# Takatsuka-Mark/Photogrammetry

Hardware: AMD Instinct MI355X
Metric: descriptor pairs matched/sec (higher is better)
Workload: dtype u8 / bits (descriptor bits expanded to fp4 +-1 for the MFMA distance: exact integers in f32 accumulators; integer keys); f32 grey; 1 GPU; BASELINE configs[2] (SURVEY 8d config 3) x 1: 64-frame 1920x1080 RGBA64 sequence(s), dewarp(shipped coeffs)+gray+FAST(T=0.1)+NMS(r=16; SURVEY 8d writes r = 20 for this config: both leave more than 4096 survivors per frame, the lists are cut to the same length either way)+BRIEF-256 per frame, all 2016 ordered image pairs per sequence through the greedy Hamming match, <=4096 keypoints per frame (fir; frames=64, image_pairs=2016, frames_per_gpu=64, image_pairs_per_gpu=2016, parallelism=frames f mod 1, image pairs p mod 1; 2 all-gathers per step (elided at N = 1), jobs_in_flight=2, rehearsal_on_one_gpu_with_gloo=False

## Files before the change

### photogrammetry_amd/csrc/k_fast.hip

```cpp
#include "pgx_internal.h"

namespace {

constexpr int TW = 64, TH = 32, HALO = 3;
constexpr int LROWS = TH + 2 * HALO;
constexpr int LSTRIDE = 72;

__global__ __launch_bounds__(256) void k_fast_planes(const float *__restrict__ gray, int W, int H, float T,
                                                     unsigned long long *__restrict__ seg, int ntx,
                                                     uint32_t *__restrict__ segcnt)
{
    __shared__ float tile[LROWS][LSTRIDE];
    __shared__ uint16_t queue[TW * TH];
    __shared__ unsigned planes[TH][3][2];
    __shared__ unsigned qcount;
    const int tx = blockIdx.x, ty = blockIdx.y, f = blockIdx.z;
    const int lane = threadIdx.x & 63, wv = threadIdx.x >> 6;
    const float *g = gray + (size_t)f * W * H;
    const int x0 = tx * TW - HALO, y0 = ty * TH - HALO;
    if (threadIdx.x < TH * 6) (&planes[0][0][0])[threadIdx.x] = 0u;
    if (threadIdx.x == 0) qcount = 0u;

    {
        constexpr int NR = (LROWS + 3) / 4;
        float v[NR], hv[NR];
#pragma unroll
        for (int k = 0; k < NR; k++) {
            const int r = wv + 4 * k;
            const int gy = y0 + r;
            const bool rowok = r < LROWS && gy >= 0 && gy < H;
            const float *grow = g + (size_t)(rowok ? gy : 0) * W;
            const int gx = x0 + lane, hx = x0 + 64 + lane;
            v[k] = (rowok && gx >= 0 && gx < W) ? grow[gx] : 0.0f;
            hv[k] = (rowok && lane < 2 * HALO && hx < W) ? grow[hx] : 0.0f;
        }
#pragma unroll
        for (int k = 0; k < NR; k++) {
            const int r = wv + 4 * k;
            if (r < LROWS) {
                tile[r][lane] = v[k];
                if (lane < 2 * HALO) tile[r][64 + lane] = hv[k];
            }
        }
    }
    __syncthreads();

    const int x = tx * TW + lane;
    const bool xin = x >= 3 && x < W - 3;
#pragma unroll 1
    for (int k = 0; k < TH / 4; k++) {
        const int ry = wv * (TH / 4) + k;
        const int y = ty * TH + ry;
        if (y >= H) break;
        bool pass = false;
        unsigned cb = 0;
        if (xin && y >= 3 && y < H - 3) {
            const float c = tile[ry + 3][lane + 3];
            const float lo = __fsub_rn(c, T), hi = __fadd_rn(c, T);
#define PGX_SIM(dx, dy) ((tile[ry + 3 + (dy)][lane + 3 + (dx)] > lo) & (tile[ry + 3 + (dy)][lane + 3 + (dx)] < hi))
            const unsigned s0 = PGX_SIM(-3, 0), s4 = PGX_SIM(0, 3), s8 = PGX_SIM(3, 0), s12 = PGX_SIM(0, -3);
#undef PGX_SIM
            pass = s0 + s4 + s8 + s12 <= 1u;
            cb = s0 | (s4 << 1) | (s8 << 2) | (s12 << 3);
        }
        const unsigned long long pm = __ballot(pass);
        if (pm) {
            unsigned base = 0;
            if (lane == 0) base = atomicAdd(&qcount, (unsigned)__popcll(pm));
            base = (unsigned)__shfl((int)base, 0);
            if (pass) queue[base + (unsigned)__popcll(pm & ((1ull << lane) - 1ull))] = (uint16_t)((ry << 10) | (lane << 4) | cb);
        }
    }
    __syncthreads();

    const unsigned nq = qcount;
    for (unsigned e = threadIdx.x; e < nq; e += 256) {
        const unsigned q = queue[e];
        const int ry = (int)(q >> 10), lx = (int)((q >> 4) & 63u);
        const float c = tile[ry + 3][lx + 3];
        const float lo = __fsub_rn(c, T), hi = __fadd_rn(c, T);
#define PGX_SIM(dx, dy) ((unsigned)((tile[ry + 3 + (dy)][lx + 3 + (dx)] > lo) & (tile[ry + 3 + (dy)][lx + 3 + (dx)] < hi)))
        unsigned S = (q & 1u) | ((q & 2u) << 3) | ((q & 4u) << 6) | ((q & 8u) << 9);
        const unsigned s1 = PGX_SIM(-3, 1);
        S |= s1 << 1;
        S |= PGX_SIM(-2, 2) << 2;
        S |= PGX_SIM(-1, 3) << 3;
        S |= PGX_SIM(1, 3) << 5;
        S |= PGX_SIM(2, 2) << 6;
        S |= PGX_SIM(3, 1) << 7;
        S |= PGX_SIM(3, -1) << 9;
        S |= PGX_SIM(2, -2) << 10;
        S |= PGX_SIM(1, -3) << 11;
        S |= PGX_SIM(-1, -3) << 13;
        S |= PGX_SIM(-2, -2) << 14;
        S |= s1 << 15;
#undef PGX_SIM
        int score = 0;
        if (S == 0u) {
            score = 16;
        } else {
            const unsigned D = ~S & 0xFFFFu;
            const unsigned dd = D | (D << 16);
            const unsigned x1 = dd & (dd >> 1);
            const unsigned x2 = x1 & (x1 >> 2);
            const unsigned x3 = x2 & (x2 >> 4);
            const unsigned t12 = x3 & (x2 >> 8);
            if (t12) {
                const unsigned t13 = t12 & (dd >> 12);
                const unsigned t14 = t13 & (dd >> 13);
                const unsigned t15 = t14 & (dd >> 14);
                score = 12 + (t13 != 0u) + (t14 != 0u) + (t15 != 0u);
            }
        }
        if (score) {
            const int code = score - 11;
            const unsigned bit = 1u << (lx & 31);
            unsigned *pw = &planes[ry][0][lx >> 5];
            if (code & 1) atomicOr(pw, bit);
            if (code & 2) atomicOr(pw + 2, bit);
            if (code & 4) atomicOr(pw + 4, bit);
        }
    }
    __syncthreads();

    if (threadIdx.x < TH) {
        const int ry = threadIdx.x, y = ty * TH + ry;
        if (y < H) {
            const unsigned long long b0 = planes[ry][0][0] | ((unsigned long long)planes[ry][0][1] << 32);
            const unsigned long long b1 = planes[ry][1][0] | ((unsigned long long)planes[ry][1][1] << 32);
            const unsigned long long b2 = planes[ry][2][0] | ((unsigned long long)planes[ry][2][1] << 32);
            unsigned long long *o = seg + (((size_t)f * H + y) * ntx + tx) * 4;
            *reinterpret_cast<ulonglong2 *>(o) = make_ulonglong2(b0, b1);
            const uint32_t cnt = (uint32_t)__popcll(b0 | b1 | b2);
            *reinterpret_cast<ulonglong2 *>(o + 2) = make_ulonglong2(b2, (unsigned long long)cnt);
            segcnt[((size_t)f * H + y) * ntx + tx] = cnt;
        }
    }
}

__global__ __launch_bounds__(1024) void k_seg_scan(int nseg, uint32_t *__restrict__ segoff, int32_t *__restrict__ n_raw,
                                                   int raw_cap, int *status)
{
    __shared__ uint32_t wsum[16];
    __shared__ uint32_t carry_s;
    const int f = blockIdx.x;
    uint32_t *so = segoff + (size_t)f * nseg;
    const int tid = threadIdx.x, lane = tid & 63, wv = tid >> 6;
    if (tid == 0) carry_s = 0;
    __syncthreads();
    for (int base = 0; base < nseg; base += 1024 * 4) {
        const int i0 = base + tid * 4;
        uint32_t c[4];
        if (i0 + 3 < nseg && (nseg & 3) == 0) {
            const uint4 v = *reinterpret_cast<const uint4 *>(so + i0);
            c[0] = v.x; c[1] = v.y; c[2] = v.z; c[3] = v.w;
        } else {
#pragma unroll
            for (int k = 0; k < 4; k++) c[k] = (i0 + k < nseg) ? so[i0 + k] : 0u;
        }
        uint32_t tsum = c[0] + c[1] + c[2] + c[3];
        uint32_t incl = tsum;
#pragma unroll
        for (int d = 1; d < 64; d <<= 1) {
            uint32_t v = __shfl_up(incl, d);
            if (lane >= d) incl += v;
        }
        if (lane == 63) wsum[wv] = incl;
        __syncthreads();
        uint32_t woff = 0;
        for (int w = 0; w < wv; w++) woff += wsum[w];
        uint32_t run = carry_s + woff + incl - tsum;
#pragma unroll
// ... 14 lines not shown
__global__ __launch_bounds__(256) void k_fast_compact(const unsigned long long *__restrict__ seg,
                                                      const uint32_t *__restrict__ segoff, int H, int ntx,
                                                      uint32_t *__restrict__ raw_xy, int32_t *__restrict__ raw_score,
                                                      int raw_cap)
{
    const int f = blockIdx.y;
    const int nseg = H * ntx;
    const int s = blockIdx.x * 256 + threadIdx.x;
    if (s >= nseg) return;
    const unsigned long long *sg = seg + ((size_t)f * nseg + s) * 4;
    const ulonglong2 p01 = *reinterpret_cast<const ulonglong2 *>(sg);
    const unsigned long long b0 = p01.x, b1 = p01.y, b2 = sg[2];
    unsigned long long any = b0 | b1 | b2;
    if (!any) return;
    uint32_t pos = segoff[(size_t)f * nseg + s];
    const int y = s / ntx, tx = s - y * ntx;
    while (any) {
        const int l = __builtin_ctzll(any);
        any &= any - 1;
        if (pos >= (uint32_t)raw_cap) break;
        const int code = (int)((b0 >> l) & 1ull) | ((int)((b1 >> l) & 1ull) << 1) | ((int)((b2 >> l) & 1ull) << 2);
        raw_xy[(size_t)f * raw_cap + pos] = ((uint32_t)y << 16) | (uint32_t)(tx * 64 + l);
        raw_score[(size_t)f * raw_cap + pos] = code + 11;
        pos++;
    }
}

}

size_t pgx_fast_seg_count(int W, int H) { return (size_t)H * ((W + TW - 1) / TW); }

void pgx_launch_fast(hipStream_t s, const float *gray, int F, int W, int H, float T,
                     unsigned long long *seg, uint32_t *segoff, int32_t *n_raw, uint32_t *raw_xy,
                     int32_t *raw_score, int raw_cap, int *status, bool compact)
{
    if (F <= 0 || W <= 0 || H <= 0) return;
    const int ntx = (W + TW - 1) / TW, nty = (H + TH - 1) / TH;
    const int nseg = H * ntx;
    hipLaunchKernelGGL(k_fast_planes, dim3(ntx, nty, F), dim3(256), 0, s, gray, W, H, T, seg, ntx, segoff);
    hipLaunchKernelGGL(k_seg_scan, dim3(F), dim3(1024), 0, s, nseg, segoff, n_raw, raw_cap, status);
    if (compact)
        hipLaunchKernelGGL(k_fast_compact, dim3((nseg + 255) / 256, F), dim3(256), 0, s, seg, segoff, H, ntx, raw_xy,
                           raw_score, raw_cap);
}
```

### photogrammetry_amd/csrc/k_image.hip

```cpp
#include "pgx_internal.h"

namespace {

__device__ __forceinline__ float gray_of(uint2 px)
{
    float r = (float)(px.x & 0xFFFFu), g = (float)(px.x >> 16), b = (float)(px.y & 0xFFFFu);
    float s = __fadd_rn(__fadd_rn(r, b), g);
    return __fdiv_rn(s, 196605.0f);
}

constexpr int FB = 4;

__device__ __forceinline__ uint2 widen8(uint32_t v)
{
    return make_uint2(__builtin_amdgcn_perm(v, v, 0x01010000u), __builtin_amdgcn_perm(v, v, 0x03030202u));
}

template <bool SRC8> struct SrcPix { using type = uint2; };
template <> struct SrcPix<true> { using type = uint32_t; };
template <bool SRC8> __device__ __forceinline__ uint2 load_px(const typename SrcPix<SRC8>::type *p);
template <> __device__ __forceinline__ uint2 load_px<false>(const uint2 *p) { return *p; }
template <> __device__ __forceinline__ uint2 load_px<true>(const uint32_t *p) { return widen8(*p); }

template <bool HAS_MAP, bool WRITE_RGBA, bool SRC8>
__global__ __launch_bounds__(256) void k_dewarp_gray(const typename SrcPix<SRC8>::type *__restrict__ rgba,
                                                     const int2 *__restrict__ map, int W, int H, int F,
                                                     float *__restrict__ gray, uint2 *__restrict__ dewarped, int *status)
{
    using Px = typename SrcPix<SRC8>::type;
    const size_t npix = (size_t)W * H;
    const int f0 = blockIdx.y * FB;
    const int nf = F - f0 < FB ? F - f0 : FB;
    const size_t ngroups = (npix + 3) / 4;
    const bool vec = (npix & 3) == 0 || F == 1;
    bool oob = false;
    for (size_t grp = (size_t)blockIdx.x * blockDim.x + threadIdx.x; grp < ngroups;
         grp += (size_t)gridDim.x * blockDim.x) {
        const size_t i0 = grp * 4;
        if (vec && i0 + 3 < npix) {
            size_t so[4];
            bool ok[4];
            if (HAS_MAP) {
                const int4 m01 = *reinterpret_cast<const int4 *>(map + i0);
                const int4 m23 = *reinterpret_cast<const int4 *>(map + i0 + 2);
                const int us[4] = {m01.x, m01.z, m23.x, m23.z};
                const int vs[4] = {m01.y, m01.w, m23.y, m23.w};
#pragma unroll
                for (int k = 0; k < 4; k++) {
                    const unsigned su = (unsigned)us[k] & 0xFFFFu, sv = (unsigned)vs[k] & 0xFFFFu;
                    ok[k] = su < (unsigned)W && sv < (unsigned)H;
                    oob |= !ok[k];
                    so[k] = ok[k] ? (size_t)sv * W + su : 0;
                }
            }
            uint2 px[FB][4];
// ... 21 lines not shown
#pragma unroll
                    for (int k = 0; k < 4; k++) if (!ok[k]) px[fb][k] = make_uint2(0, 0);
                }
                if (gray) {
                    const float4 g4 = make_float4(gray_of(px[fb][0]), gray_of(px[fb][1]), gray_of(px[fb][2]), gray_of(px[fb][3]));
                    *reinterpret_cast<float4 *>(gray + (size_t)(f0 + fb) * npix + i0) = g4;
                }
                if (WRITE_RGBA) {
                    uint2 *dout = dewarped + (size_t)(f0 + fb) * npix;
                    *reinterpret_cast<uint4 *>(dout + i0) = make_uint4(px[fb][0].x, px[fb][0].y, px[fb][1].x, px[fb][1].y);
                    *reinterpret_cast<uint4 *>(dout + i0 + 2) = make_uint4(px[fb][2].x, px[fb][2].y, px[fb][3].x, px[fb][3].y);
                }
            }
        } else {
            for (size_t i = i0; i < npix && i < i0 + 4; i++) {
                size_t o = i;
                bool okk = true;
                if (HAS_MAP) {
                    const int2 m = map[i];
                    const unsigned su = (unsigned)m.x & 0xFFFFu, sv = (unsigned)m.y & 0xFFFFu;
                    okk = su < (unsigned)W && sv < (unsigned)H;
                    oob |= !okk;
                    o = okk ? (size_t)sv * W + su : 0;
                }
                for (int fb = 0; fb < nf; fb++) {
                    const uint2 p = okk ? load_px<SRC8>(rgba + (size_t)(f0 + fb) * npix + o) : make_uint2(0, 0);
                    if (gray) gray[(size_t)(f0 + fb) * npix + i] = gray_of(p);
                    if (WRITE_RGBA) dewarped[(size_t)(f0 + fb) * npix + i] = p;
                }
            }
        }
    }
    if (HAS_MAP && oob) atomicOr(status, (int)PGX_ST_OOB_SOURCE);
}

__device__ __forceinline__ int32_t trunc_to_int_dev(double v)
{
    if (!(v > -2147483649.0 && v < 2147483648.0)) return INT32_MIN;
    return (int32_t)v;
}

__device__ __forceinline__ double cbrt_signed_dev(double n)
{
    const double sgn = (double)((n > 0) - (n < 0));
    return pow(fabs(n), 1.0 / 3.0) * sgn;
}

__global__ __launch_bounds__(256) void k_dewarp_map(int W, int H, double k0, double k1, double k2, double k3, double k4,
                                                    int2 *__restrict__ map, int *status)
{
    const size_t i = (size_t)blockIdx.x * 256 + threadIdx.x;
    if (i >= (size_t)W * H) return;
    const int v = (int)(i / W), u = (int)(i - (size_t)v * W);
    const double x0 = W / 2.0, y0 = H / 2.0;
    const int x = trunc_to_int_dev(u - x0), y = trunc_to_int_dev(v - y0);
    const int rd2 = x * x + y * y;
    const double rd = sqrt((double)rd2);
    const double den = rd * k4 - k1;
    const double a2 = (rd * k3 - k0) / den, a1 = (rd * k2 - 1) / den, a0 = rd / den;
    const double Q = (3 * a1 - a2 * a2) / 9.0;
    const double R = (9.0 * a2 * a1 - 27 * a0 - 2 * a2 * a2 * a2) / 54.0;
    const double Q3 = Q * Q * Q;
    const double D = Q3 + R * R;
    const double shift = -a2 / 3.0;
    const double nan = __longlong_as_double(0x7FF8000000000000ll);
    double r0 = nan, r1 = nan, r2 = nan;
// ... 22 lines not shown
        if (kept[0] > kept[1]) { const double t = kept[0]; kept[0] = kept[1]; kept[1] = t; }
    }
    const double root = n == 3 ? kept[1] : kept[0];
    const double theta = atan2((double)y, (double)x);
    map[i] = make_int2(trunc_to_int_dev(root * cos(theta) + x0), trunc_to_int_dev(root * sin(theta) + y0));
}

}

void pgx_launch_dewarp_gray(hipStream_t s, const void *rgba, int src8, const int32_t *map_uv, int F, int W, int H,
                            float *gray, uint16_t *dewarped, int *status)
{
    if (F <= 0 || W <= 0 || H <= 0) return;
    const size_t ngroups = ((size_t)W * H + 3) / 4;
    unsigned gx = (unsigned)((ngroups + 255) / 256);
    const unsigned ny = (unsigned)((F + FB - 1) / FB);
    const unsigned cap = 512u / ny > 32u ? 512u / ny : 32u;
    if (gx > cap) gx = cap;
    dim3 grid(gx, (unsigned)((F + FB - 1) / FB)), block(256);
    const int2 *map = reinterpret_cast<const int2 *>(map_uv);
    uint2 *dw = reinterpret_cast<uint2 *>(dewarped);
#define PGX_DG(M, WR, S8) hipLaunchKernelGGL((k_dewarp_gray<M, WR, S8>), grid, block, 0, s, \
                                             reinterpret_cast<const SrcPix<S8>::type *>(rgba), map, W, H, F, gray, dw, status)
    if (src8) {
        if (map) { if (dw) PGX_DG(true, true, true); else PGX_DG(true, false, true); }
        else { if (dw) PGX_DG(false, true, true); else PGX_DG(false, false, true); }
    } else {
        if (map) { if (dw) PGX_DG(true, true, false); else PGX_DG(true, false, false); }
        else { if (dw) PGX_DG(false, true, false); else PGX_DG(false, false, false); }
    }
#undef PGX_DG
}

void pgx_launch_dewarp_map(hipStream_t s, int W, int H, const double *k, int32_t *map_uv, int *status)
{
    const size_t npix = (size_t)W * H;
    hipLaunchKernelGGL(k_dewarp_map, dim3((unsigned)((npix + 255) / 256)), dim3(256), 0, s, W, H, k[0], k[1], k[2], k[3], k[4],
                       reinterpret_cast<int2 *>(map_uv), status);
}
```

### photogrammetry_amd/csrc/pgx_api.hip

```cpp
#include "pgx_trackgraph.h"
#include "pgx_brief_plan.h"

#include <atomic>
#include <cmath>
#include <cstdarg>
#include <cstdio>
#include <new>
#include <cstring>
#include <cstdlib>

#define PGX_VERSION_STR "pgx 0.1 (gfx950)"

static thread_local std::string tl_err;
static thread_local const pgx_ctx *tl_err_ctx = nullptr;
static thread_local unsigned long long tl_err_id = 0;
static std::atomic<unsigned long long> g_ctx_ids{0};

void pgx_note_error(pgx_ctx *c, const std::string &msg)
{
    tl_err = msg;
    tl_err_ctx = c;
    tl_err_id = c ? c->id : 0;
    if (c) {
        std::lock_guard<std::mutex> g(c->err_mu);
// ... 139 lines not shown
    HIPCHK(c, c->ws_rawxy.ensure((size_t)F * raw_cap * 4));
    HIPCHK(c, c->ws_rawscore.ensure((size_t)F * raw_cap * 4));
    HIPCHK(c, c->ws_nms.ensure((size_t)F * nms_stride));
    const int kp_eff = c->kp_cap <= cap ? c->kp_cap : cap;
    HIPCHK(c, c->ws_order.ensure((size_t)F * kp_eff * 4));
    HIPCHK(c, c->ws_nkept.ensure((size_t)F * 4));
    if (pl.n_levels > 1) {
        HIPCHK(c, c->ws_pyr_cnt.ensure((size_t)16 * F * 4));
        if (pl.n_run > 1) {
            const size_t slots = (size_t)(pl.n_run - 1) * F * kp_eff;
            HIPCHK(c, c->ws_pyr_a.ensure((size_t)F * pl.dims[1][0] * pl.dims[1][1] * 4));
            if (pl.n_run > 2) HIPCHK(c, c->ws_pyr_b.ensure((size_t)F * pl.dims[2][0] * pl.dims[2][1] * 4));
            HIPCHK(c, c->ws_pyr_kp.ensure(slots * sizeof(pgx_keypoint)));
            HIPCHK(c, c->ws_pyr_desc.ensure(slots * c->words * 4));
            if (c->steer_on) HIPCHK(c, c->ws_pyr_bins.ensure(slots * 4));
        }
    }
    return PGX_OK;
}

namespace {

PgxSteer steer_of(const pgx_ctx *c, int32_t *d_bins = nullptr)
{
    return PgxSteer{c->d_steer_pairs.as<int32_t>(), c->d_steer_plans.as<int32_t>(), c->d_steer_dirs.as<int32_t>(), c->steer_B,
                    c->steer_R, d_bins};
}

void enqueue_from_gray(pgx_ctx *c, const float *gray, int F, int W, int H, int kp_eff, bool kp_soft, pgx_keypoint *d_kp,
                       uint32_t *d_desc, int32_t *d_counts, int32_t *d_nraw, int out_stride, int32_t *d_bins)
{
    const int raw_cap = c->raw_cap;
    const size_t nms_stride = pgx_nms_ws_bytes(W, H, c->radius, raw_cap, true);
    {
        ProfScope ps(c, "fast");
        pgx_launch_fast(c->stream, gray, F, W, H, c->threshold, c->ws_seg.as<unsigned long long>(),
                        c->ws_segoff.as<uint32_t>(), d_nraw, c->ws_rawxy.as<uint32_t>(),
                        c->ws_rawscore.as<int32_t>(), raw_cap, c->d_status,
                        !pgx_nms_fills_raw_lists(W, H, c->radius, raw_cap));
    }
    {
        ProfScope ps(c, "nms");
        pgx_launch_nms(c->stream, c->ws_rawxy.as<uint32_t>(), c->ws_rawscore.as<int32_t>(), d_nraw, F, raw_cap, W, H,
                       c->radius, c->ws_nms.p, nms_stride, c->ws_order.as<uint32_t>(), c->ws_nkept.as<int32_t>(),
                       kp_eff, c->d_status, c->ws_seg.as<unsigned long long>(), c->ws_segoff.as<uint32_t>(), kp_soft);
    }
    {
        ProfScope ps(c, "brief");
        const PgxSteer st = steer_of(c, d_bins);
        pgx_launch_brief(c->stream, gray, F, W, H, c->ws_rawxy.as<uint32_t>(), c->ws_rawscore.as<int32_t>(), raw_cap,
                         c->ws_order.as<uint32_t>(), c->ws_nkept.as<int32_t>(), kp_eff, c->d_pairs.as<int32_t>(), c->d_plan.as<int32_t>(), c->P,
                         d_kp, d_desc, d_counts, out_stride, c->steer_on ? &st : nullptr);
    }
}

int enqueue_detect_bins(pgx_ctx *c, const uint16_t *d_rgba, int F, int W, int H, pgx_keypoint *d_kp, uint32_t *d_desc,
                        int32_t *d_counts, int32_t *d_nraw, int cap, int32_t *d_bins, int32_t *d_origin = nullptr,
                        int32_t *d_stats = nullptr)
{
    const int rcp = pgx_prepare_detect(c, F, W, H, cap);
    if (rcp != PGX_OK) return rcp;
    if (F <= 0) return PGX_OK;
    const bool kp_soft = c->kp_cap <= cap;
    const int kp_eff = kp_soft ? c->kp_cap : cap;

    float *gray = c->ws_gray.as<float>();
    {
        ProfScope ps(c, "dewarp_gray");
        pgx_launch_dewarp_gray(c->stream, d_rgba, c->src8, c->map_set ? c->d_map.as<int32_t>() : nullptr, F, W, H, gray,
                               nullptr, c->d_status);
    }
    if (c->pyr_levels <= 1) {
        enqueue_from_gray(c, gray, F, W, H, kp_eff, kp_soft, d_kp, d_desc, d_counts, d_nraw, cap, d_bins);
    } else {
        const PyrPlan pl = pyr_plan(c, W, H);
        int32_t *lvl_counts = c->ws_pyr_cnt.as<int32_t>(), *lvl_nraw = lvl_counts + (size_t)8 * F;
        const size_t lvl_slots = (size_t)F * kp_eff;
        int32_t *tmp_bins = d_bins ? c->ws_pyr_bins.as<int32_t>() : nullptr;
        enqueue_from_gray(c, gray, F, W, H, kp_eff, kp_soft, d_kp, d_desc, lvl_counts, lvl_nraw, cap, d_bins);
        const float *src = gray;
        for (int l = 1; l < pl.n_run; l++) {
            float *dst = (l & 1) ? c->ws_pyr_a.as<float>() : c->ws_pyr_b.as<float>();
            {
                ProfScope ps(c, "pyramid");
                pgx_launch_pyr_down(c->stream, src, F, pl.dims[l - 1][0], pl.dims[l - 1][1], dst, pl.dims[l][0], pl.dims[l][1],
                                    c->pyr_step);
            }
            enqueue_from_gray(c, dst, F, pl.dims[l][0], pl.dims[l][1], kp_eff, kp_soft,
                              c->ws_pyr_kp.as<pgx_keypoint>() + (l - 1) * lvl_slots,
                              c->ws_pyr_desc.as<uint32_t>() + (l - 1) * lvl_slots * c->words, lvl_counts + (size_t)l * F,
                              lvl_nraw + (size_t)l * F, kp_eff, tmp_bins ? tmp_bins + (l - 1) * lvl_slots : nullptr);
            src = dst;
        }
        {
            ProfScope ps(c, "pyramid_append");
            pgx_launch_pyr_append(c->stream, c->ws_pyr_kp.as<pgx_keypoint>(), c->ws_pyr_desc.as<uint32_t>(), tmp_bins, lvl_counts,
                                  lvl_nraw, F, kp_eff, c->words, pl.n_levels, pl.n_run, W, H, pl.scale, d_kp, d_desc, d_bins,
                                  d_counts, d_nraw, d_origin, d_stats, cap, c->d_status);
        }
    }
    HIPCHK(c, hipEventRecord(c->ev_stage[PGX_STAGE_DETECT], c->stream));
    HIPCHK(c, hipGetLastError());
    return PGX_OK;
}
// ... 112 lines not shown
    if (strncmp(prop.gcnArchName, "gfx950", 6) != 0) {
        fprintf(stderr, "pgx: device %d is %s; this library is built for gfx950 only\n", device, prop.gcnArchName);
        return PGX_E_HIP;
    }
    pgx_ctx *c = new (std::nothrow) pgx_ctx();
    if (!c) return PGX_E_HIP;
    c->device = device;
    c->id = ++g_ctx_ids;
    if (hipStreamCreateWithFlags(&c->own_stream, hipStreamNonBlocking) != hipSuccess ||
        hipEventCreateWithFlags(&c->ev_stage[0], hipEventDisableTiming) != hipSuccess ||
        hipEventCreateWithFlags(&c->ev_stage[1], hipEventDisableTiming) != hipSuccess ||
        hipEventCreateWithFlags(&c->ev_stage[2], hipEventDisableTiming) != hipSuccess ||
        hipEventCreateWithFlags(&c->ev_stage[3], hipEventDisableTiming) != hipSuccess ||
        hipMalloc(reinterpret_cast<void **>(&c->d_status), 256) != hipSuccess ||
        hipHostMalloc(reinterpret_cast<void **>(&c->h_status), 64, hipHostMallocDefault) != hipSuccess ||
        hipMemset(c->d_status, 0, 256) != hipSuccess) {
        pgx_ctx_destroy(c);
        return PGX_E_HIP;
    }
    c->stream = c->own_stream;
    *out = c;
    return PGX_OK;
}

void pgx_ctx_destroy(pgx_ctx *c)
{
    if (!c) return;
    (void)hipSetDevice(c->device);
    if (c->stream) (void)hipStreamSynchronize(c->stream);
    if (c->comm) (void)pgx_comm_destroy(c);
    for (auto &kv : c->prof)
        for (auto &ev : kv.second.pending) { (void)hipEventDestroy(ev.first); (void)hipEventDestroy(ev.second); }
    for (hipEvent_t ev : c->ev_pool) (void)hipEventDestroy(ev);
    DevBuf *bufs[] = {&c->d_pairs, &c->d_plan, &c->d_steer_pairs, &c->d_steer_plans, &c->d_steer_dirs, &c->d_map, &c->ws_gray, &c->ws_seg, &c->ws_segoff, &c->ws_nraw, &c->ws_rawxy,
                      &c->ws_rawscore, &c->ws_nms, &c->ws_order, &c->ws_nkept, &c->st_a, &c->st_b, &c->st_c,
                      &c->st_d, &c->st_e, &c->st_f, &c->ws_pose, &c->ws_tracks, &c->ws_tracks_split, &c->ws_agree, &c->ws_matchn[0], &c->ws_matchn[1], &c->ws_matchn[2], &c->ws_knn, &c->ws_guided, &c->ws_tri, &c->ws_ba, &c->ws_reg, &c->ws_ver, &c->ws_init, &c->ws_cns, &c->ws_vocab,
                      &c->ws_pyr_a, &c->ws_pyr_b, &c->ws_pyr_kp, &c->ws_pyr_desc, &c->ws_pyr_bins, &c->ws_pyr_cnt};
    for (DevBuf *b : bufs) b->release();
    c->pin_in.release();
    c->pin_out.release();
    if (c->d_status) (void)hipFree(c->d_status);
    if (c->h_status) (void)hipHostFree(c->h_status);
    for (int k = 0; k < 3; k++) {
        if (c->mstream[k]) (void)hipStreamDestroy(c->mstream[k]);
        if (c->ev_wide[k]) (void)hipEventDestroy(c->ev_wide[k]);
        if (c->ev_rows[k]) (void)hipEventDestroy(c->ev_rows[k]);
        if (c->ev_fin[k]) (void)hipEventDestroy(c->ev_fin[k]);
        if (c->ev_join[k]) (void)hipEventDestroy(c->ev_join[k]);
    }
    if (c->ev_in) (void)hipEventDestroy(c->ev_in);
    for (int k = 0; k < 4; k++) if (c->ev_stage[k]) (void)hipEventDestroy(c->ev_stage[k]);
    if (c->own_stream) (void)hipStreamDestroy(c->own_stream);
    delete c;
}

const char *pgx_last_error(pgx_ctx *c)
{
    if (!c) return "null context";
    if (tl_err_ctx == c && tl_err_id == c->id) return tl_err.c_str();
    static thread_local std::string copy;
    {
        std::lock_guard<std::mutex> g(c->err_mu);
        copy = c->err;
    }
    return copy.c_str();
}

int pgx_set_stream(pgx_ctx *c, void *hip_stream)
{
    if (!c) return PGX_E_BADARG;
    Lock l(c);
    c->cfg_epoch++;
    HIPCHK(c, hipStreamSynchronize(c->stream));
    c->stream = hip_stream ? reinterpret_cast<hipStream_t>(hip_stream) : c->own_stream;
    return PGX_OK;
}

int pgx_check_status(pgx_ctx *c)
{
    if (!c) return PGX_E_BADARG;
    Lock l(c);
    return sync_status(c);
}

int pgx_set_dewarp_map(pgx_ctx *c, const int32_t *uv, int W, int H)
{
    if (!c) return PGX_E_BADARG;
    Lock l(c);
    c->cfg_epoch++;
    if (!uv) { c->map_set = false; c->mapW = c->mapH = 0; return PGX_OK; }
    if (dims_ok(c, W, H, "map dimensions must fit ushort") != PGX_OK) return PGX_E_BADARG;
    const size_t bytes = (size_t)W * H * 8;
    HIPCHK(c, hipStreamSynchronize(c->stream));
    HIPCHK(c, c->d_map.ensure(bytes + 32));
    HIPCHK(c, hipMemcpy(c->d_map.p, uv, bytes, hipMemcpyHostToDevice));
    c->mapW = W; c->mapH = H; c->map_set = true;
    return PGX_OK;
}

int pgx_set_dewarp_coeffs(pgx_ctx *c, int W, int H, const double *coeffs, int ncoeffs)
{
    if (!c || !coeffs) return c ? fail(c, PGX_E_BADARG, "null pointer") : PGX_E_BADARG;
    Lock l(c);
    c->cfg_epoch++;
    if (ncoeffs != 5) return fail(c, PGX_E_BADARG, "You must pass exactly 5 distortion coefficients (ArgumentException)");
    if (dims_ok(c, W, H, "map dimensions must fit ushort") != PGX_OK) return PGX_E_BADARG;
    const size_t bytes = (size_t)W * H * 8;
    HIPCHK(c, hipStreamSynchronize(c->stream));
    HIPCHK(c, c->d_map.ensure(bytes + 32));
    pgx_launch_dewarp_map(c->stream, W, H, coeffs, c->d_map.as<int32_t>(), c->d_status);
    HIPCHK(c, hipGetLastError());
    c->mapW = W; c->mapH = H; c->map_set = true;
    return sync_status(c);
}

int pgx_get_dewarp_map(pgx_ctx *c, int32_t *uv_out, int W, int H)
{
    if (!c || !uv_out) return c ? fail(c, PGX_E_BADARG, "null pointer") : PGX_E_BADARG;
    Lock l(c);
    if (!c->map_set) return fail(c, PGX_E_NOT_CONFIGURED, "no dewarp map is set");
    if (W != c->mapW || H != c->mapH) return fail(c, PGX_E_DIM_MISMATCH, "map is %dx%d, asked for %dx%d", c->mapW, c->mapH, W, H);
    HIPCHK(c, hipStreamSynchronize(c->stream));
    HIPCHK(c, hipMemcpy(uv_out, c->d_map.p, (size_t)W * H * 8, hipMemcpyDeviceToHost));
    return PGX_OK;
}

int pgx_set_brief_pairs(pgx_ctx *c, const int32_t *pairs, int P)
{
    if (!c) return PGX_E_BADARG;
    Lock l(c);
    c->cfg_epoch++;
    if (!pairs || P <= 0 || P > 4064) return fail(c, PGX_E_BADARG, "P must be in [1, 4064]");
    HIPCHK(c, hipStreamSynchronize(c->stream));
    HIPCHK(c, c->d_pairs.ensure((size_t)P * 16));
    HIPCHK(c, hipMemcpy(c->d_pairs.p, pairs, (size_t)P * 16, hipMemcpyHostToDevice));
    if (P == PGX_PLAN_PAIRS) {
        int32_t plan[PGX_PLAN_WORDS];
        pgx_build_brief_plan(pairs, plan);
        HIPCHK(c, c->d_plan.ensure(sizeof plan));
        HIPCHK(c, hipMemcpy(c->d_plan.p, plan, sizeof plan, hipMemcpyHostToDevice));
    }
    c->P = P; c->words = (P + 31) / 32; c->pairs_set = true;
    c->steer_on = false;
    return PGX_OK;
}
// ... 1371 lines not shown
```

### photogrammetry_amd/csrc/pgx_internal.h

```cpp
#pragma once

#include <hip/hip_runtime.h>
#include <stdint.h>

#include <map>
#include <mutex>
#include <string>
#include <type_traits>
#include <utility>
#include <vector>

#include "../../include/pgx.h"

#define PGX_ST_OOB_SOURCE 1u
#define PGX_ST_RAW_CAP    2u
#define PGX_ST_KP_CAP     4u
#define PGX_ST_EMPTY_SET  8u
#define PGX_ST_INTERNAL   16u
#define PGX_ST_BADARG     32u
#define PGX_ST_DUP_FRAME  64u
#define PGX_ST_TRI_CAP    128u
#define PGX_ST_TRI_NODE   256u
#define PGX_ST_TRI_DUP    512u
#define PGX_ST_BA_CAP     1024u
// ... 51 lines not shown
    }
    void release() { if (p) (void)hipHostFree(p); p = nullptr; cap = 0; }
    template <class T> T *as() const { return reinterpret_cast<T *>(p); }
};

struct ProfEntry {
    std::vector<std::pair<hipEvent_t, hipEvent_t>> pending;
    int launches = 0;
    double total_ms = 0.0;
};

struct pgx_ctx {
    int device = 0;
    hipStream_t own_stream = nullptr;
    hipStream_t stream = nullptr;
    std::mutex mu;
    std::string err;
    std::mutex err_mu;

    float threshold = 0.f;
    int radius = 0;
    bool params_set = false;
    int P = 0, words = 0;
    bool pairs_set = false;
    DevBuf d_pairs;
    DevBuf d_plan;
    bool steer_on = false;
    int steer_B = 0, steer_R = 0;
    DevBuf d_steer_pairs, d_steer_plans, d_steer_dirs;
    int pyr_levels = 1, pyr_step = 0;
    int mapW = 0, mapH = 0;
    bool map_set = false;
    DevBuf d_map;
    int raw_cap = 1 << 17;
    int kp_cap = 1 << PGX_IDX_BITS;
    int match_chunk = 2048;
    int src8 = 0;

    int *d_status = nullptr;
    int *h_status = nullptr;

    DevBuf ws_gray, ws_seg, ws_segoff, ws_nraw, ws_rawxy, ws_rawscore, ws_nms, ws_order, ws_nkept;
    DevBuf ws_pyr_a, ws_pyr_b, ws_pyr_kp, ws_pyr_desc, ws_pyr_bins, ws_pyr_cnt;
    DevBuf st_a, st_b, st_c, st_d, st_e, st_f;
    PinBuf pin_in, pin_out;
    DevBuf ws_matchn[3];
    DevBuf ws_pose, ws_tracks;
    DevBuf ws_tracks_split;
    DevBuf ws_knn;
    DevBuf ws_guided;
    DevBuf ws_tri;
    DevBuf ws_ba;
    DevBuf ws_reg;
    DevBuf ws_cns;
    DevBuf ws_ver;
    DevBuf ws_vocab;
    DevBuf ws_init;
    hipStream_t mstream[3] = {nullptr, nullptr, nullptr};
    hipEvent_t ev_in = nullptr, ev_wide[3] = {nullptr, nullptr, nullptr}, ev_rows[3] = {nullptr, nullptr, nullptr},
               ev_fin[3] = {nullptr, nullptr, nullptr}, ev_join[3] = {nullptr, nullptr, nullptr};
    hipEvent_t ev_stage[4] = {nullptr, nullptr, nullptr, nullptr};
    hipEvent_t match_gate = nullptr;

    void *comm = nullptr;
    int comm_rank = 0, comm_world = 1;
    std::string comm_agreed;
// ... 30 lines not shown

void pgx_note_error(pgx_ctx *c, const std::string &msg);

struct ProfScope {
    pgx_ctx *c;
    ProfEntry *e = nullptr;
    hipEvent_t a = nullptr, b = nullptr;
    hipStream_t st;
    bool attach;
    ProfScope(pgx_ctx *ctx, const char *name, hipStream_t s = nullptr, bool attach_to_kernel = false)
        : c(ctx), st(s ? s : ctx->stream), attach(attach_to_kernel)
    {
        if (!name || !c->prof_on || (!c->prof_only.empty() && c->prof_only != name)) return;
        e = &c->prof[name];
        auto take = [&](hipEvent_t &ev) {
            if (!c->ev_pool.empty()) { ev = c->ev_pool.back(); c->ev_pool.pop_back(); return true; }
            return hipEventCreate(&ev) == hipSuccess;
        };
        if (!take(a) || !take(b)) { e = nullptr; a = b = nullptr; return; }
        if (!attach) (void)hipEventRecord(a, st);
    }
    ~ProfScope()
    {
        if (!e) return;
        if (!attach) (void)hipEventRecord(b, st);
        e->pending.emplace_back(a, b);
    }
};


void pgx_launch_dewarp_gray(hipStream_t s, const void *rgba, int src8, const int32_t *map_uv, int F, int W, int H,
                            float *gray, uint16_t *dewarped, int *status);
void pgx_launch_dewarp_map(hipStream_t s, int W, int H, const double *k , int32_t *map_uv, int *status);

size_t pgx_fast_seg_count(int W, int H);
void pgx_launch_fast(hipStream_t s, const float *gray, int F, int W, int H, float T,
                     unsigned long long *seg , uint32_t *segoff ,
                     int32_t *n_raw , uint32_t *raw_xy ,
                     int32_t *raw_score , int raw_cap, int *status,
                     bool compact = true );

size_t pgx_nms_ws_bytes(int W, int H, int radius, int n_cap, bool planes);
bool pgx_nms_fills_raw_lists(int W, int H, int radius, int n_cap);
void pgx_launch_nms(hipStream_t s, uint32_t *raw_xy, int32_t *raw_score, const int32_t *n_raw,
                    int F, int n_cap, int W, int H, int radius, void *ws, size_t ws_stride,
                    uint32_t *order , int32_t *n_kept , int kp_cap, int *status,
                    const unsigned long long *seg = nullptr ,
                    const uint32_t *segoff = nullptr,
                    bool kp_soft = false );
hipError_t pgx_launch_nms_sync(hipStream_t s, const uint32_t *raw_xy, const int32_t *raw_score, const int32_t *n_raw,
                               int n_cap, int W, int H, int radius, void *ws, size_t ws_stride, uint32_t *order,
                               int32_t *n_kept, int kp_cap, int *status);

struct PgxSteer {
    const int32_t *pairs_rot;
    const int32_t *plans;
    const int32_t *dirs;
    int B, R;
    int32_t *bins_out;
};

void pgx_launch_brief(hipStream_t s, const float *gray, int F, int W, int H,
                      const uint32_t *raw_xy, const int32_t *raw_score, int raw_cap,
                      const uint32_t *order, const int32_t *n_kept, int kp_cap ,
                      const int32_t *pairs, const int32_t *plan , int P,
                      pgx_keypoint *kp_out, uint32_t *desc_out, int32_t *counts_out, int out_stride ,
                      const PgxSteer *steer = nullptr);
void pgx_launch_brief_list(hipStream_t s, const float *gray, int W, int H, const pgx_keypoint *kps, int n,
                           const int32_t *pairs, const int32_t *plan, int P, uint32_t *desc_out, const PgxSteer *steer = nullptr);

void pgx_launch_steer(hipStream_t s, const float *gray, int F, int W, int H, const uint32_t *raw_xy, const int32_t *raw_score,
                      int raw_cap, const uint32_t *order, const int32_t *n_kept, int kp_cap, const PgxSteer &st, int P,
                      pgx_keypoint *kp_out, uint32_t *desc_out, int32_t *counts_out, int out_stride);
// ... 113 lines not shown
```

Measured before the change: 5084 billion descriptor pairs/s.

## Fuse dewarp-gray into FAST tile kernel with precomputed gather plan

Replaces the separate dewarp_gray pass followed by FAST with a single kernel. It gathers dewarped source pixels straight into the FAST shared tile, converts them to grey, writes the grey image for later stages, and runs the FAST test on the tile. A precomputed 32-bit gather plan, built once when the map is set, replaces the per-frame int2 map decode. Tiles are remapped across XCDs and grouped by frame. This removes one full grey-image read back into FAST and one kernel launch, at the cost of gathering halo pixels redundantly and a forced register cap of 16 VGPRs that may cause spills.

```diff
diff --git a/photogrammetry_amd/csrc/k_fast.hip b/photogrammetry_amd/csrc/k_fast.hip
--- a/photogrammetry_amd/csrc/k_fast.hip
+++ b/photogrammetry_amd/csrc/k_fast.hip
@@ -1,48 +1,18 @@
 #include "pgx_internal.h"
+#include "pgx_pixel.h"
 
 namespace {
 
 constexpr int TW = 64, TH = 32, HALO = 3;
 constexpr int LROWS = TH + 2 * HALO;
 constexpr int LSTRIDE = 72;
-
-__global__ __launch_bounds__(256) void k_fast_planes(const float *__restrict__ gray, int W, int H, float T,
-                                                     unsigned long long *__restrict__ seg, int ntx,
-                                                     uint32_t *__restrict__ segcnt)
-{
-    __shared__ float tile[LROWS][LSTRIDE];
-    __shared__ uint16_t queue[TW * TH];
-    __shared__ unsigned planes[TH][3][2];
-    __shared__ unsigned qcount;
-    const int tx = blockIdx.x, ty = blockIdx.y, f = blockIdx.z;
+constexpr int NR = (LROWS + 3) / 4;
+
+__device__ __forceinline__ void fast_tile(const float (*tile)[LSTRIDE], uint16_t *queue, unsigned (*planes)[3][2],
+                                          unsigned *qcount, int tx, int ty, int f, int W, int H, float T,
+                                          unsigned long long *__restrict__ seg, int ntx, uint32_t *__restrict__ segcnt)
+{
     const int lane = threadIdx.x & 63, wv = threadIdx.x >> 6;
-    const float *g = gray + (size_t)f * W * H;
-    const int x0 = tx * TW - HALO, y0 = ty * TH - HALO;
-    if (threadIdx.x < TH * 6) (&planes[0][0][0])[threadIdx.x] = 0u;
-    if (threadIdx.x == 0) qcount = 0u;
-
-    {
-        constexpr int NR = (LROWS + 3) / 4;
-        float v[NR], hv[NR];
-#pragma unroll
-        for (int k = 0; k < NR; k++) {
-            const int r = wv + 4 * k;
-            const int gy = y0 + r;
-            const bool rowok = r < LROWS && gy >= 0 && gy < H;
-            const float *grow = g + (size_t)(rowok ? gy : 0) * W;
-            const int gx = x0 + lane, hx = x0 + 64 + lane;
-            v[k] = (rowok && gx >= 0 && gx < W) ? grow[gx] : 0.0f;
-            hv[k] = (rowok && lane < 2 * HALO && hx < W) ? grow[hx] : 0.0f;
-        }
-#pragma unroll
-        for (int k = 0; k < NR; k++) {
-            const int r = wv + 4 * k;
-            if (r < LROWS) {
-                tile[r][lane] = v[k];
-                if (lane < 2 * HALO) tile[r][64 + lane] = hv[k];
-            }
-        }
-    }
     __syncthreads();
 
     const int x = tx * TW + lane;
@@ -66,14 +36,14 @@
         const unsigned long long pm = __ballot(pass);
         if (pm) {
             unsigned base = 0;
-            if (lane == 0) base = atomicAdd(&qcount, (unsigned)__popcll(pm));
+            if (lane == 0) base = atomicAdd(qcount, (unsigned)__popcll(pm));
             base = (unsigned)__shfl((int)base, 0);
             if (pass) queue[base + (unsigned)__popcll(pm & ((1ull << lane) - 1ull))] = (uint16_t)((ry << 10) | (lane << 4) | cb);
         }
     }
     __syncthreads();
 
-    const unsigned nq = qcount;
+    const unsigned nq = *qcount;
     for (unsigned e = threadIdx.x; e < nq; e += 256) {
         const unsigned q = queue[e];
         const int ry = (int)(q >> 10), lx = (int)((q >> 4) & 63u);
@@ -138,6 +108,135 @@
     }
 }
 
+__global__ __launch_bounds__(256) void k_fast_planes(const float *__restrict__ gray, int W, int H, float T,
+                                                     unsigned long long *__restrict__ seg, int ntx,
+                                                     uint32_t *__restrict__ segcnt)
+{
+    __shared__ float tile[LROWS][LSTRIDE];
+    __shared__ uint16_t queue[TW * TH];
+    __shared__ unsigned planes[TH][3][2];
+    __shared__ unsigned qcount;
+    const int tx = blockIdx.x, ty = blockIdx.y, f = blockIdx.z;
+    const int lane = threadIdx.x & 63, wv = threadIdx.x >> 6;
+    const float *g = gray + (size_t)f * W * H;
+    const int x0 = tx * TW - HALO, y0 = ty * TH - HALO;
+    if (threadIdx.x < TH * 6) (&planes[0][0][0])[threadIdx.x] = 0u;
+    if (threadIdx.x == 0) qcount = 0u;
+
+    {
+        float v[NR], hv[NR];
+#pragma unroll
+        for (int k = 0; k < NR; k++) {
+            const int r = wv + 4 * k;
+            const int gy = y0 + r;
+            const bool rowok = r < LROWS && gy >= 0 && gy < H;
+            const float *grow = g + (size_t)(rowok ? gy : 0) * W;
+            const int gx = x0 + lane, hx = x0 + 64 + lane;
+            v[k] = (rowok && gx >= 0 && gx < W) ? grow[gx] : 0.0f;
+            hv[k] = (rowok && lane < 2 * HALO && hx < W) ? grow[hx] : 0.0f;
+        }
+#pragma unroll
+        for (int k = 0; k < NR; k++) {
+            const int r = wv + 4 * k;
+            if (r < LROWS) {
+                tile[r][lane] = v[k];
+                if (lane < 2 * HALO) tile[r][64 + lane] = hv[k];
+            }
+        }
+    }
+    fast_tile(tile, queue, planes, &qcount, tx, ty, f, W, H, T, seg, ntx, segcnt);
+}
+
+constexpr int FG = 8;
+constexpr int GB = NR / 2;
+constexpr int HALO_N = LROWS * 2 * HALO;
+
+template <bool HAS_MAP, bool SRC8>
+__attribute__((amdgpu_num_vgpr(16)))
+__global__ __launch_bounds__(256) void k_dewarp_fast(const typename SrcPix<SRC8>::type *__restrict__ rgba,
+                                                     const uint32_t *__restrict__ plan, const uint32_t *__restrict__ plan_oob,
+                                                     int W, int H, int F, float T, float *__restrict__ gray,
+                                                     unsigned long long *__restrict__ seg, int ntx, int nty,
+                                                     uint32_t *__restrict__ segcnt, int *status)
+{
+    using Px = typename SrcPix<SRC8>::type;
+    __shared__ float tile[LROWS][LSTRIDE];
+    __shared__ uint16_t queue[TW * TH];
+    __shared__ unsigned planes[TH][3][2];
+    __shared__ unsigned qcount;
+    if (HAS_MAP && blockIdx.x == 0 && threadIdx.x == 0 && *plan_oob) atomicOr(status, (int)PGX_ST_OOB_SOURCE);
+    const int nxy = ntx * nty, ntile = nxy * F;
+    const int per_xcd = (ntile + 7) >> 3;
+    const int id = (int)(blockIdx.x & 7u) * per_xcd + (int)(blockIdx.x >> 3);
+    if (id >= ntile) return;
+    int f, txy;
+    {
+        const int FF = (F / FG) * FG;
+        if (id < nxy * FF) {
+            const int g = id / (nxy * FG), r = id - g * (nxy * FG);
+            txy = r / FG;
+            f = g * FG + r % FG;
+        } else {
+            const int r = id - nxy * FF, nl = F - FF;
+            txy = r / nl;
+            f = FF + r % nl;
+        }
+    }
+    const int ty = txy / ntx, tx = txy - ty * ntx;
+    const int lane = threadIdx.x & 63, wv = threadIdx.x >> 6;
+    const int x0 = tx * TW - HALO, y0 = ty * TH - HALO;
+    const size_t npix = (size_t)W * H;
+    const Px *src = rgba + (size_t)f * npix;
+    float *gout = gray + (size_t)f * npix;
+    if (threadIdx.x < TH * 6) (&planes[0][0][0])[threadIdx.x] = 0u;
+    if (threadIdx.x == 0) qcount = 0u;
+
+    const int gx = x0 + lane;
+    const int hr = (int)threadIdx.x / (2 * HALO), hc = TW + (int)threadIdx.x % (2 * HALO);
+    const int hx = x0 + hc, hy = y0 + hr;
+    const bool hin = threadIdx.x < HALO_N && hy >= 0 && hy < H && hx < W;
+    auto offset_of = [&](int k) {
+        const int r = wv + 4 * k, gy = y0 + r;
+        uint32_t o = PGX_GATHER_OOB;
+        if (r < LROWS && gy >= 0 && gy < H && gx >= 0 && gx < W) {
+            o = (uint32_t)gy * (uint32_t)W + (uint32_t)gx;
+            if (HAS_MAP) o = plan[o];
+        }
+        return o;
+    };
+    auto pixel_at = [&](uint32_t o) { return o != PGX_GATHER_OOB ? load_px<SRC8>(src + o) : make_uint2(0u, 0u); };
+    auto put = [&](int k, uint2 p) {
+        const int r = wv + 4 * k, gy = y0 + r;
+        if (r < LROWS) {
+            const float g = gray_of(p);
+            tile[r][lane] = g;
+            if (lane >= HALO && r >= HALO && r < TH + HALO && gx < W && gy < H) gout[(uint32_t)gy * (uint32_t)W + (uint32_t)gx] = g;
+        }
+    };
+#pragma unroll
+    for (int k0 = 0; k0 < NR; k0 += GB) {
+        uint32_t off[GB], hoff = PGX_GATHER_OOB;
+        uint2 px[GB], hpx = make_uint2(0u, 0u);
+#pragma unroll
+        for (int j = 0; j < GB; j++) off[j] = offset_of(k0 + j);
+        if (k0 == 0 && hin) {
+            hoff = (uint32_t)hy * (uint32_t)W + (uint32_t)hx;
+            if (HAS_MAP) hoff = plan[hoff];
+        }
+#pragma unroll
+        for (int j = 0; j < GB; j++) px[j] = pixel_at(off[j]);
+        if (k0 == 0) hpx = pixel_at(hoff);
+#pragma unroll
+        for (int j = 0; j < GB; j++) put(k0 + j, px[j]);
+        if (k0 == 0 && threadIdx.x < HALO_N) {
+            const float g = gray_of(hpx);
+            tile[hr][hc] = g;
+            if (hc < TW + HALO && hr >= HALO && hr < TH + HALO && hin) gout[(uint32_t)hy * (uint32_t)W + (uint32_t)hx] = g;
+        }
+    }
+    fast_tile(tile, queue, planes, &qcount, tx, ty, f, W, H, T, seg, ntx, segcnt);
+}
+
 __global__ __launch_bounds__(1024) void k_seg_scan(int nseg, uint32_t *__restrict__ segoff, int32_t *__restrict__ n_raw,
                                                    int raw_cap, int *status)
 {
@@ -218,14 +317,29 @@
 
 void pgx_launch_fast(hipStream_t s, const float *gray, int F, int W, int H, float T,
                      unsigned long long *seg, uint32_t *segoff, int32_t *n_raw, uint32_t *raw_xy,
-                     int32_t *raw_score, int raw_cap, int *status, bool compact)
+                     int32_t *raw_score, int raw_cap, int *status, bool compact, bool planes)
 {
     if (F <= 0 || W <= 0 || H <= 0) return;
     const int ntx = (W + TW - 1) / TW, nty = (H + TH - 1) / TH;
     const int nseg = H * ntx;
-    hipLaunchKernelGGL(k_fast_planes, dim3(ntx, nty, F), dim3(256), 0, s, gray, W, H, T, seg, ntx, segoff);
+    if (planes)
+        hipLaunchKernelGGL(k_fast_planes, dim3(ntx, nty, F), dim3(256), 0, s, gray, W, H, T, seg, ntx, segoff);
     hipLaunchKernelGGL(k_seg_scan, dim3(F), dim3(1024), 0, s, nseg, segoff, n_raw, raw_cap, status);
     if (compact)
         hipLaunchKernelGGL(k_fast_compact, dim3((nseg + 255) / 256, F), dim3(256), 0, s, seg, segoff, H, ntx, raw_xy,
                            raw_score, raw_cap);
 }
+
+void pgx_launch_dewarp_fast(hipStream_t s, const void *rgba, int src8, const uint32_t *plan, const uint32_t *plan_oob, int F,
+                            int W, int H, float T, float *gray, unsigned long long *seg, uint32_t *segoff, int *status)
+{
+    if (F <= 0 || W <= 0 || H <= 0) return;
+    const int ntx = (W + TW - 1) / TW, nty = (H + TH - 1) / TH;
+    const int ntile = ntx * nty * F;
+    const dim3 grid((unsigned)(8 * ((ntile + 7) / 8))), block(256);
+#define PGX_DF(M, S8) hipLaunchKernelGGL((k_dewarp_fast<M, S8>), grid, block, 0, s, reinterpret_cast<const SrcPix<S8>::type *>(rgba), \
+                                         plan, plan_oob, W, H, F, T, gray, seg, ntx, nty, segoff, status)
+    if (src8) { if (plan) PGX_DF(true, true); else PGX_DF(false, true); }
+    else { if (plan) PGX_DF(true, false); else PGX_DF(false, false); }
+#undef PGX_DF
+}
diff --git a/photogrammetry_amd/csrc/k_image.hip b/photogrammetry_amd/csrc/k_image.hip
--- a/photogrammetry_amd/csrc/k_image.hip
+++ b/photogrammetry_amd/csrc/k_image.hip
@@ -1,26 +1,9 @@
 #include "pgx_internal.h"
+#include "pgx_pixel.h"
 
 namespace {
 
-__device__ __forceinline__ float gray_of(uint2 px)
-{
-    float r = (float)(px.x & 0xFFFFu), g = (float)(px.x >> 16), b = (float)(px.y & 0xFFFFu);
-    float s = __fadd_rn(__fadd_rn(r, b), g);
-    return __fdiv_rn(s, 196605.0f);
-}
-
 constexpr int FB = 4;
-
-__device__ __forceinline__ uint2 widen8(uint32_t v)
-{
-    return make_uint2(__builtin_amdgcn_perm(v, v, 0x01010000u), __builtin_amdgcn_perm(v, v, 0x03030202u));
-}
-
-template <bool SRC8> struct SrcPix { using type = uint2; };
-template <> struct SrcPix<true> { using type = uint32_t; };
-template <bool SRC8> __device__ __forceinline__ uint2 load_px(const typename SrcPix<SRC8>::type *p);
-template <> __device__ __forceinline__ uint2 load_px<false>(const uint2 *p) { return *p; }
-template <> __device__ __forceinline__ uint2 load_px<true>(const uint32_t *p) { return widen8(*p); }
 
 template <bool HAS_MAP, bool WRITE_RGBA, bool SRC8>
 __global__ __launch_bounds__(256) void k_dewarp_gray(const typename SrcPix<SRC8>::type *__restrict__ rgba,
@@ -108,6 +91,18 @@
         }
     }
     if (HAS_MAP && oob) atomicOr(status, (int)PGX_ST_OOB_SOURCE);
+}
+
+__global__ __launch_bounds__(256) void k_dewarp_plan(const int2 *__restrict__ map, int W, int H, uint32_t *__restrict__ plan,
+                                                     uint32_t *__restrict__ flag)
+{
+    const size_t i = (size_t)blockIdx.x * 256 + threadIdx.x;
+    if (i >= (size_t)W * H) return;
+    const int2 m = map[i];
+    const unsigned su = (unsigned)m.x & 0xFFFFu, sv = (unsigned)m.y & 0xFFFFu;
+    const bool ok = su < (unsigned)W && sv < (unsigned)H;
+    plan[i] = ok ? sv * (unsigned)W + su : PGX_GATHER_OOB;
+    if (!ok) atomicOr(flag, 1u);
 }
 
 __device__ __forceinline__ int32_t trunc_to_int_dev(double v)
@@ -196,6 +191,14 @@
 #undef PGX_DG
 }
 
+void pgx_launch_dewarp_plan(hipStream_t s, const int32_t *map_uv, int W, int H, uint32_t *plan, uint32_t *flag)
+{
+    const size_t npix = (size_t)W * H;
+    (void)hipMemsetAsync(flag, 0, 4, s);
+    hipLaunchKernelGGL(k_dewarp_plan, dim3((unsigned)((npix + 255) / 256)), dim3(256), 0, s, reinterpret_cast<const int2 *>(map_uv), W,
+                       H, plan, flag);
+}
+
 void pgx_launch_dewarp_map(hipStream_t s, int W, int H, const double *k, int32_t *map_uv, int *status)
 {
     const size_t npix = (size_t)W * H;
diff --git a/photogrammetry_amd/csrc/pgx_api.hip b/photogrammetry_amd/csrc/pgx_api.hip
--- a/photogrammetry_amd/csrc/pgx_api.hip
+++ b/photogrammetry_amd/csrc/pgx_api.hip
@@ -195,12 +195,18 @@
 {
     const int raw_cap = c->raw_cap;
     const size_t nms_stride = pgx_nms_ws_bytes(W, H, c->radius, raw_cap, true);
+    const void *rgba = c->fuse_rgba;
+    c->fuse_rgba = nullptr;
     {
         ProfScope ps(c, "fast");
+        if (rgba)
+            pgx_launch_dewarp_fast(c->stream, rgba, c->src8, c->map_set ? c->d_gather.as<uint32_t>() : nullptr,
+                                   c->map_set ? c->gather_flag() : nullptr, F, W, H, c->threshold, const_cast<float *>(gray),
+                                   c->ws_seg.as<unsigned long long>(), c->ws_segoff.as<uint32_t>(), c->d_status);
         pgx_launch_fast(c->stream, gray, F, W, H, c->threshold, c->ws_seg.as<unsigned long long>(),
                         c->ws_segoff.as<uint32_t>(), d_nraw, c->ws_rawxy.as<uint32_t>(),
                         c->ws_rawscore.as<int32_t>(), raw_cap, c->d_status,
-                        !pgx_nms_fills_raw_lists(W, H, c->radius, raw_cap));
+                        !pgx_nms_fills_raw_lists(W, H, c->radius, raw_cap), rgba == nullptr);
     }
     {
         ProfScope ps(c, "nms");
@@ -228,11 +234,7 @@
     const int kp_eff = kp_soft ? c->kp_cap : cap;
 
     float *gray = c->ws_gray.as<float>();
-    {
-        ProfScope ps(c, "dewarp_gray");
-        pgx_launch_dewarp_gray(c->stream, d_rgba, c->src8, c->map_set ? c->d_map.as<int32_t>() : nullptr, F, W, H, gray,
-                               nullptr, c->d_status);
-    }
+    c->fuse_rgba = d_rgba;
     if (c->pyr_levels <= 1) {
         enqueue_from_gray(c, gray, F, W, H, kp_eff, kp_soft, d_kp, d_desc, d_counts, d_nraw, cap, d_bins);
     } else {
@@ -411,7 +413,7 @@
     for (auto &kv : c->prof)
         for (auto &ev : kv.second.pending) { (void)hipEventDestroy(ev.first); (void)hipEventDestroy(ev.second); }
     for (hipEvent_t ev : c->ev_pool) (void)hipEventDestroy(ev);
-    DevBuf *bufs[] = {&c->d_pairs, &c->d_plan, &c->d_steer_pairs, &c->d_steer_plans, &c->d_steer_dirs, &c->d_map, &c->ws_gray, &c->ws_seg, &c->ws_segoff, &c->ws_nraw, &c->ws_rawxy,
+    DevBuf *bufs[] = {&c->d_pairs, &c->d_plan, &c->d_steer_pairs, &c->d_steer_plans, &c->d_steer_dirs, &c->d_map, &c->d_gather, &c->ws_gray, &c->ws_seg, &c->ws_segoff, &c->ws_nraw, &c->ws_rawxy,
                       &c->ws_rawscore, &c->ws_nms, &c->ws_order, &c->ws_nkept, &c->st_a, &c->st_b, &c->st_c,
                       &c->st_d, &c->st_e, &c->st_f, &c->ws_pose, &c->ws_tracks, &c->ws_tracks_split, &c->ws_agree, &c->ws_matchn[0], &c->ws_matchn[1], &c->ws_matchn[2], &c->ws_knn, &c->ws_guided, &c->ws_tri, &c->ws_ba, &c->ws_reg, &c->ws_ver, &c->ws_init, &c->ws_cns, &c->ws_vocab,
                       &c->ws_pyr_a, &c->ws_pyr_b, &c->ws_pyr_kp, &c->ws_pyr_desc, &c->ws_pyr_bins, &c->ws_pyr_cnt};
@@ -467,13 +469,21 @@
     if (!c) return PGX_E_BADARG;
     Lock l(c);
     c->cfg_epoch++;
-    if (!uv) { c->map_set = false; c->mapW = c->mapH = 0; return PGX_OK; }
+    if (!uv) {
+        HIPCHK(c, hipStreamSynchronize(c->stream));
+        c->d_gather.release();
+        c->map_set = false; c->mapW = c->mapH = 0;
+        return PGX_OK;
+    }
     if (dims_ok(c, W, H, "map dimensions must fit ushort") != PGX_OK) return PGX_E_BADARG;
     const size_t bytes = (size_t)W * H * 8;
     HIPCHK(c, hipStreamSynchronize(c->stream));
     HIPCHK(c, c->d_map.ensure(bytes + 32));
+    HIPCHK(c, c->d_gather.ensure(bytes / 2 + 4));
     HIPCHK(c, hipMemcpy(c->d_map.p, uv, bytes, hipMemcpyHostToDevice));
     c->mapW = W; c->mapH = H; c->map_set = true;
+    pgx_launch_dewarp_plan(c->stream, c->d_map.as<int32_t>(), W, H, c->d_gather.as<uint32_t>(), c->gather_flag());
+    HIPCHK(c, hipGetLastError());
     return PGX_OK;
 }
 
@@ -487,9 +497,11 @@
     const size_t bytes = (size_t)W * H * 8;
     HIPCHK(c, hipStreamSynchronize(c->stream));
     HIPCHK(c, c->d_map.ensure(bytes + 32));
+    HIPCHK(c, c->d_gather.ensure(bytes / 2 + 4));
     pgx_launch_dewarp_map(c->stream, W, H, coeffs, c->d_map.as<int32_t>(), c->d_status);
-    HIPCHK(c, hipGetLastError());
     c->mapW = W; c->mapH = H; c->map_set = true;
+    pgx_launch_dewarp_plan(c->stream, c->d_map.as<int32_t>(), W, H, c->d_gather.as<uint32_t>(), c->gather_flag());
+    HIPCHK(c, hipGetLastError());
     return sync_status(c);
 }
 
diff --git a/photogrammetry_amd/csrc/pgx_internal.h b/photogrammetry_amd/csrc/pgx_internal.h
--- a/photogrammetry_amd/csrc/pgx_internal.h
+++ b/photogrammetry_amd/csrc/pgx_internal.h
@@ -107,6 +107,9 @@
     int mapW = 0, mapH = 0;
     bool map_set = false;
     DevBuf d_map;
+    DevBuf d_gather;
+    uint32_t *gather_flag() const { return d_gather.as<uint32_t>() + (size_t)mapW * mapH; }
+    const void *fuse_rgba = nullptr;
     int raw_cap = 1 << 17;
     int kp_cap = 1 << PGX_IDX_BITS;
     int match_chunk = 2048;
@@ -203,13 +206,17 @@
 void pgx_launch_dewarp_gray(hipStream_t s, const void *rgba, int src8, const int32_t *map_uv, int F, int W, int H,
                             float *gray, uint16_t *dewarped, int *status);
 void pgx_launch_dewarp_map(hipStream_t s, int W, int H, const double *k , int32_t *map_uv, int *status);
+void pgx_launch_dewarp_plan(hipStream_t s, const int32_t *map_uv, int W, int H, uint32_t *plan, uint32_t *flag);
 
 size_t pgx_fast_seg_count(int W, int H);
 void pgx_launch_fast(hipStream_t s, const float *gray, int F, int W, int H, float T,
                      unsigned long long *seg , uint32_t *segoff ,
                      int32_t *n_raw , uint32_t *raw_xy ,
                      int32_t *raw_score , int raw_cap, int *status,
-                     bool compact = true );
+                     bool compact = true ,
+                     bool planes = true );
+void pgx_launch_dewarp_fast(hipStream_t s, const void *rgba, int src8, const uint32_t *plan, const uint32_t *plan_oob, int F,
+                            int W, int H, float T, float *gray, unsigned long long *seg, uint32_t *segoff, int *status);
 
 size_t pgx_nms_ws_bytes(int W, int H, int radius, int n_cap, bool planes);
 bool pgx_nms_fills_raw_lists(int W, int H, int radius, int n_cap);
diff --git a/photogrammetry_amd/csrc/pgx_pixel.h b/photogrammetry_amd/csrc/pgx_pixel.h
--- /dev/null
+++ b/photogrammetry_amd/csrc/pgx_pixel.h
@@ -0,0 +1,23 @@
+#pragma once
+#include <stdint.h>
+#include <hip/hip_runtime.h>
+
+__device__ __forceinline__ float gray_of(uint2 px)
+{
+    float r = (float)(px.x & 0xFFFFu), g = (float)(px.x >> 16), b = (float)(px.y & 0xFFFFu);
+    float s = __fadd_rn(__fadd_rn(r, b), g);
+    return __fdiv_rn(s, 196605.0f);
+}
+
+__device__ __forceinline__ uint2 widen8(uint32_t v)
+{
+    return make_uint2(__builtin_amdgcn_perm(v, v, 0x01010000u), __builtin_amdgcn_perm(v, v, 0x03030202u));
+}
+
+template <bool SRC8> struct SrcPix { using type = uint2; };
+template <> struct SrcPix<true> { using type = uint32_t; };
+template <bool SRC8> __device__ __forceinline__ uint2 load_px(const typename SrcPix<SRC8>::type *p);
+template <> __device__ __forceinline__ uint2 load_px<false>(const uint2 *p) { return *p; }
+template <> __device__ __forceinline__ uint2 load_px<true>(const uint32_t *p) { return widen8(*p); }
+
+#define PGX_GATHER_OOB 0xFFFFFFFFu
```

After: 5182 billion descriptor pairs/s (median of 6 runs). 1.02x the previous value.
